# dblanm/gnn-manip

Measured on AMD Instinct MI355X. Metric: rollout steps/sec (N particles, 10 MP steps, hidden=128), higher is better.
Workload: dtype f32; 1 GPU; north_star target: N=100k dense synthetic scene, conn_r=0.015, max_neighbours=20, hidden=128, 10 MP steps; n_particles=100000, hidden=128, edges_last_step=1966056, k_steps=6, candidates_per_gpu=1, parallelism=candidate-parallel x1

## Files before the change

gnn_manip_amd/csrc/blocks_dev.h:

```cpp
#pragma once
#include "common.h"
#include "hedge.h"

namespace gm {

constexpr int kBlockEdges = 32;
__host__ __device__ inline int edge_blocks_padded(int n_edges) { return ((n_edges + kBlockEdges - 1) / kBlockEdges + 3) & ~3; }

#if defined(__HIPCC__)
__device__ inline void edge_blocks_plan(const int* __restrict__ in_ptr, int n_nodes, const int* n_per_dev, int n_per_host,
                                        EdgeBlockHeader* tab, int* gblk, int max_graphs) {
    int n_per = n_per_dev ? *n_per_dev : n_per_host;
    if (n_per <= 0) n_per = n_nodes > 0 ? n_nodes : 1;
    int G = (n_nodes + n_per - 1) / n_per;
    if (G > max_graphs) G = max_graphs;
    int pb = 0;
    for (int g = 0; g < G; ++g) {
        const int lo = g * n_per, hi = min(n_nodes, (g + 1) * n_per);
        gblk[g] = pb;
        pb += edge_blocks_padded(in_ptr[hi] - in_ptr[lo]);
    }
    gblk[G] = pb;
    tab->n_blocks = pb;
    tab->n_groups = pb / 4;
    tab->n_graphs = G;
    tab->n_per_graph = n_per;
    tab->n_stitch = 0;
}

__device__ inline void edge_blocks_fill(const int* __restrict__ in_ptr, const int* __restrict__ dst, int n_nodes, EdgeBlockHeader* tab,
                                        const int* __restrict__ gblk, int2* blk, int2* seg, int* __restrict__ head, int* __restrict__ stitch,
                                        int* __restrict__ stitch_list, int t, int nt) {
    constexpr int BE = kBlockEdges;
    const int nblk = tab->n_blocks, G = tab->n_graphs, n_per = tab->n_per_graph;
    for (int b = t; b < nblk; b += nt) {
        int lo = 0, hi = G;
        while (hi - lo > 1) {
            const int mid = (lo + hi) >> 1;
            if (gblk[mid] <= b) lo = mid; else hi = mid;
        }
        const int g = lo, j = b - gblk[g];
        const int e0 = in_ptr[g * n_per], e1 = in_ptr[min(n_nodes, (g + 1) * n_per)];
        const int start = min(e0 + j * BE, e1);
        const int cnt = min(BE, e1 - start);
        const int fl = ((j & 3) == 0 ? 1 : 0) | ((j & 3) == 3 ? 2 : 0);
        blk[b] = make_int2(start, cnt | (fl << 8));
        {
// ... 8 lines not shown
                else is_last = (j & 3) == 3 || cnt < BE || start + cnt >= e1 || dst[start + cnt] != d;
                if (is_last) last |= 1u << n;
            }
            seg[b] = make_int2((int)cont, (int)last);
        }
        if ((j & 3) == 0) {
            int h = -1;
            if (cnt > 0 && start > e0 && dst[start - 1] == dst[start]) h = dst[start];
            head[b >> 2] = h;
            if (h >= 0) {
                const int ps = start - 4 * BE;
                const bool prev_is_head = j >= 4 && dst[ps] == h && ps > e0 && dst[ps - 1] == h;
                if (!prev_is_head) {
                    stitch[h] = b >> 2;
                    stitch_list[atomicAdd(&tab->n_stitch, 1)] = h;
                }
            }
        }
    }
}
#endif

}
```

gnn_manip_amd/csrc/common.h:

```cpp
#pragma once
#include <hip/hip_runtime.h>
#include <stdint.h>
#include <stdio.h>
#include <string.h>
#include <mutex>
#include "../../include/gnn_manip_hip.h"

namespace gm {

void set_error(const char* fmt, ...);

#define GM_HIP_CHECK(expr)                                                                  \
    do {                                                                                    \
        hipError_t _e = (expr);                                                             \
        if (_e != hipSuccess) {                                                             \
            gm::set_error("%s failed: %s (%s:%d)", #expr, hipGetErrorString(_e), __FILE__,  \
                          __LINE__);                                                        \
            return GM_ERR_HIP;                                                              \
        }                                                                                   \
    } while (0)

#define GM_REQUIRE(cond, code, ...)          \
    do {                                     \
        if (!(cond)) {                       \
// ... 90 lines not shown
    size_t bytes;
};
int max_cells_for(int64_t n);
GraphWs carve_graph(void* ws, int64_t n, int max_nb);

struct CsrHeader {
    int n_edges;
    int error_flags;
    int flow;
    int pad;
};
struct CsrWs {
    CsrHeader* hdr;
    int* in_ptr;
    int* cursor;
    int* dst;
    int* src;
    int* eid;
    int* scan_in;
    int* sort_tmp;
    int64_t cap;
    int* blocks;
    size_t bytes;
};
CsrWs carve_csr(void* ws, int64_t n, int64_t cap);

enum ProfKind : int { PROF_EDGE = 0, PROF_NODE = 1, PROF_GRAPH = 2, PROF_ENC = 3, PROF_REST = 4, PROF_KINDS = 5 };
constexpr int PROF_MAX = 4096;
struct ProfState {
    int mask = 0;
// ... 114 lines not shown
```

gnn_manip_amd/csrc/graph.hip:

```cpp
#include <stdarg.h>
#include "common.h"
#include "hedge.h"
#include "blocks_dev.h"

namespace gm {

static thread_local char g_err[512] = "";
void set_error(const char* fmt, ...) {
    va_list ap;
    va_start(ap, fmt);
    vsnprintf(g_err, sizeof(g_err), fmt, ap);
    va_end(ap);
}
const char* last_error() { return g_err; }

ProfState::~ProfState() {
    for (int k = 0; k < PROF_KINDS; ++k) {
        if (!start[k]) continue;
        for (int i = 0; i < PROF_MAX; ++i) { (void)hipEventDestroy(start[k][i]); (void)hipEventDestroy(stop[k][i]); }
        delete[] start[k];
        delete[] stop[k];
    }
}

// ... 153 lines not shown
int graph_clear_jobs(StepClear& c, const GraphWs& g, int64_t n) {
    c.gh = g.hdr;
    int rc = c.add(g.cell_start, (long long)g.max_cells + 1, 0);
    if (rc == GM_OK) rc = c.add(g.cell_cursor, g.max_cells, 0);
    if (rc == GM_OK) rc = c.add(g.cnt + n, 1, 0);
    if (rc == GM_OK) rc = c.add(g.scan_cells, (long long)scan_state_ints((int64_t)g.max_cells + 1), 0);
    if (rc == GM_OK) rc = c.add(g.scan_cnt, (long long)scan_state_ints(n + 1), 0);
    return rc;
}
int csr_clear_jobs(StepClear& c, const CsrWs& w, int64_t n, int flow) {
    c.ch = w.hdr;
    c.flow = flow;
    int rc = c.add(w.in_ptr, n + 1, 0);
    if (rc == GM_OK) rc = c.add(w.scan_in, (long long)scan_state_ints(n + 1), 0);
    if (rc == GM_OK) rc = c.add(carve_edge_blocks(w.blocks, n, w.cap).stitch, n, -1);
    return rc;
}

int max_cells_for(int64_t n) {
    int64_t c = 2 * n;
    if (c < 32768) c = 32768;
    if (c > (1 << 22)) c = (1 << 22);
    return (int)c;
}

GraphWs carve_graph(void* ws, int64_t n, int max_nb) {
    GraphWs g;
    Carver c(ws);
    g.max_cells = max_cells_for(n);
    g.hdr = c.take<GraphHeader>(1);
// ... 3 lines not shown
    g.sorted = c.take<float4>(n);
    g.cnt = c.take<int>(n + 1);
    g.out_ptr = c.take<int>(n + 1);
    g.nbr = c.take<int>((size_t)n * max_nb);
    g.scan_cells = c.take<int>(scan_state_ints((int64_t)g.max_cells + 1));
    g.scan_cnt = c.take<int>(scan_state_ints(n + 1));
    g.bytes = c.used();
    return g;
}

CsrWs carve_csr(void* ws, int64_t n, int64_t cap) {
    CsrWs w;
    Carver c(ws);
    w.hdr = c.take<CsrHeader>(1);
    w.in_ptr = c.take<int>(n + 1);
    w.cursor = c.take<int>(n + 1);
    w.dst = c.take<int>(cap);
    w.src = c.take<int>(cap);
    w.eid = c.take<int>(cap);
    w.scan_in = c.take<int>(scan_state_ints(n + 1));
    w.sort_tmp = c.take<int>(2 * (size_t)cap);
    w.cap = cap;
    w.blocks = c.take<int>(edge_blocks_ints(n, cap));
    w.bytes = c.used();
    return w;
}

__device__ __forceinline__ unsigned f2ord(float f) {
    unsigned u = __float_as_uint(f);
    return (u & 0x80000000u) ? ~u : (u | 0x80000000u);
}
// ... 379 lines not shown
}

constexpr int SEG_LPS = 8;
constexpr int SEG_PER_WG = 256 / SEG_LPS;
constexpr int SEG_CAP = 96;
constexpr int SEG_STRIDE = SEG_CAP + 1;
struct BlockTabArgs {
    const int* dst;
    EdgeBlockHeader* hdr;
    const int* gblk;
    int2* blk;
    int2* seg;
    int* head;
    int* stitch;
    int* stitch_list;
    int n_tab;
};
__global__ void __launch_bounds__(256) segment_sort_kernel(const int* __restrict__ in_ptr, int64_t n,
                                                            int* __restrict__ src, int* __restrict__ eid,
                                                            CsrHeader* hdr, const float* __restrict__ pos,
                                                            int64_t pos_stride, float conn_r, float* __restrict__ edge_attr, int flow,
                                                            int* __restrict__ tmp_eid, int* __restrict__ tmp_src, BlockTabArgs bt) {
    __shared__ int se[SEG_PER_WG * SEG_STRIDE];
    __shared__ int ss[SEG_PER_WG * SEG_STRIDE];
    __shared__ int s_long[SEG_PER_WG];
    if ((int)blockIdx.x < bt.n_tab) {
        edge_blocks_fill(in_ptr, bt.dst, (int)n, bt.hdr, bt.gblk, bt.blk, bt.seg, bt.head, bt.stitch, bt.stitch_list,
                         (int)blockIdx.x * 256 + (int)threadIdx.x, bt.n_tab * 256);
        return;
    }
    const int wg = (int)blockIdx.x - bt.n_tab;
    const int tid = threadIdx.x, sub = tid & (SEG_LPS - 1), sl = tid / SEG_LPS;
    const int64_t i = (int64_t)wg * SEG_PER_WG + sl;
    if (i == 0 && sub == 0) hdr->n_edges = in_ptr[n];
    const bool active = i < n;
    const int b = active ? in_ptr[i] : 0, e = active ? in_ptr[i + 1] : 0;
    const int len = e - b;
    int* le = se + sl * SEG_STRIDE;
    int* ls = ss + sl * SEG_STRIDE;
    const bool small = len <= SEG_CAP;
    if (small)
        for (int a = sub; a < len; a += SEG_LPS) {
// ... 207 lines not shown
namespace {
int csr_tail(const GraphWs& g, int64_t n, int K, const CsrWs& c, const float* pos, int64_t pos_stride, float conn_r, float* edge_attr,
             int flow, bool with_cnt_scan, hipStream_t s) {
    const int64_t cap = n * K;
    const unsigned nb = (unsigned)cdiv(cap, 256);
    int* slot = c.sort_tmp;
    ScanJob sj[2] = {{c.in_ptr, c.in_ptr, (long long)n + 1, nullptr, c.scan_in},
                     {g.cnt, g.out_ptr, (long long)n + 1, &g.hdr->n_edges, g.scan_cnt}};
    int rc = scan_lookback(sj, with_cnt_scan ? 2 : 1, s);
    if (rc != GM_OK) return rc;
    const EdgeBlocks t = carve_edge_blocks(c.blocks, n, cap);
    hipLaunchKernelGGL(fill_graph_kernel, dim3(nb), dim3(256), 0, s, g.cnt, g.out_ptr, g.nbr, n, K, c.in_ptr,
                       slot, cap, flow, c.dst, c.src, c.eid, c.hdr, &g.hdr->n_per_graph, t.hdr, t.gblk);
    int gb = (int)cdiv(cdiv(cap, kBlockEdges) + 8, 256);
    gb = gb < 1 ? 1 : (gb > 512 ? 512 : gb);
    const BlockTabArgs bt{c.dst, t.hdr, t.gblk, t.blk, t.seg, t.head, t.stitch, t.stitch_list, gb};
    hipLaunchKernelGGL(segment_sort_kernel, dim3((unsigned)cdiv(n, SEG_PER_WG) + (unsigned)gb), dim3(256), 0, s, c.in_ptr, n, c.src, c.eid, c.hdr,
                       pos, pos_stride, conn_r, edge_attr, flow, c.sort_tmp, c.sort_tmp + c.cap, bt);
    GM_LAUNCH_CHECK();
    return GM_OK;
}
}

int csr_from_graph_with_features(const void* graph_ws, int64_t n, int K, void* csr_ws, size_t csr_ws_bytes, const float* pos,
                                 int64_t pos_stride, float conn_r, float* edge_attr, int flow, hipStream_t stream) {
    GM_REQUIRE(graph_ws && csr_ws, GM_ERR_INVALID_ARGUMENT, "gm_csr_from_graph: null pointer");
    GM_REQUIRE(flow == 0 || flow == 1, GM_ERR_INVALID_ARGUMENT, "gm_csr_from_graph: flow must be 0 or 1");
    const int64_t cap = n * K;
    GraphWs g = carve_graph(const_cast<void*>(graph_ws), n, K);
    CsrWs c = carve_csr(csr_ws, n, cap);
    GM_REQUIRE(csr_ws_bytes >= c.bytes, GM_ERR_WORKSPACE, "gm_csr_from_graph: workspace %zu < %zu", csr_ws_bytes, c.bytes);
// ... 55 lines not shown
        if (rc == GM_OK) rc = launch_step_clear(clr, s);
        if (rc != GM_OK) return rc;
    }
    if (e > 0) {
        unsigned nb = (unsigned)cdiv(e, 256);
        hipLaunchKernelGGL(indeg_ei_kernel, dim3(nb), dim3(256), 0, s, ei, n, e, flow, c.in_ptr, c.hdr);
        const ScanJob sj{c.in_ptr, c.in_ptr, (long long)n + 1, nullptr, c.scan_in};
        int rc = scan_lookback(&sj, 1, s);
        if (rc != GM_OK) return rc;
        hipLaunchKernelGGL(fill_ei_kernel, dim3(nb), dim3(256), 0, s, ei, n, e, flow, c.in_ptr, c.cursor, c.dst, c.src, c.eid, c.hdr);
    }
    if (n > 0)
        hipLaunchKernelGGL(segment_sort_kernel, dim3((unsigned)cdiv(n, SEG_PER_WG)), dim3(256), 0, s, c.in_ptr, n, c.src, c.eid, c.hdr, nullptr, 3, 1.f, nullptr, 0, c.sort_tmp, c.sort_tmp + c.cap, BlockTabArgs{});
    GM_LAUNCH_CHECK();
    if (!with_blocks) return GM_OK;
    return build_edge_blocks(c.in_ptr, c.dst, n, nullptr, (int)n, carve_edge_blocks(c.blocks, n, e), s);
}
}

extern "C" {

int gm_csr_header_status(const int32_t* header_host, int64_t* n_edges_host) {
    GM_REQUIRE(header_host, GM_ERR_INVALID_ARGUMENT, "gm_csr_header_status: null pointer");
    CsrHeader h;
    memcpy(&h, header_host, sizeof(h));
    if (n_edges_host) *n_edges_host = h.n_edges;
    GM_REQUIRE(!(h.error_flags & ERRF_BAD_EDGE_INDEX), GM_ERR_DATA, "edge_index entry out of range [0, n_nodes)");
    GM_REQUIRE(!(h.error_flags & ERRF_CAPACITY), GM_ERR_DATA, "edge capacity exceeded");
    GM_REQUIRE(!(h.error_flags & ERRF_SPLIT_RANGE), GM_ERR_DATA,
               "fp16 split range exceeded: a feature, latent or hidden activation of the last forward over this edge structure reached "
               "|x| >= 65504 in a matrix-pipe operand image (include/gnn_manip_hip.h, numeric domain); its results are not valid");
// ... 14 lines not shown
```

gnn_manip_amd/csrc/hedge.h:

```cpp
#pragma once
#include "common.h"
#include "mlp.h"

namespace gm {

struct EdgeBlockHeader {
    int n_blocks;
    int n_groups;
    int n_graphs;
    int n_per_graph;
    int n_stitch;
    int pad[3];
};
struct EdgeBlocks {
    EdgeBlockHeader* hdr;
    int* gblk;
    int2* blk;
    int2* seg;
    int* head;
    int* stitch;
    int* stitch_list;
    int64_t max_blocks;
};
size_t edge_blocks_ints(int64_t n_nodes, int64_t edge_capacity);
constexpr int kSinkRows = 1024;
size_t edge_groups_max(int64_t n_nodes, int64_t edge_capacity);
EdgeBlocks carve_edge_blocks(int* base, int64_t n_nodes, int64_t edge_capacity);
int build_edge_blocks(const int* in_ptr, const int* dst, int64_t n_nodes, const int* n_per_graph_dev, int n_per_graph_host, const EdgeBlocks& t, hipStream_t s);

constexpr int kPackH3Max = 16;
struct PackH3Job {
    const float* W1;
    int W1_col0;
    int W1_ld;
    const float* W2;
    const float* W3;
    const float* b1;
    const float* b2;
    const float* b3;
    const float* gamma;
    const float* beta;
    float* dst;
    int enc_k1;
};
size_t h3_image_floats();
int pack_h3(const PackH3Job* jobs, int n, hipStream_t s);

int launch_edge_sys(const EdgeArgs& a, const EdgeBlocks& t, int64_t edge_capacity, hipStream_t s);
inline const float* edge_sys_p_scale(const float* h3_image) { return h3_image; }

struct NodeSysArgs {
    const float* h;
    const float* agg;
    const float* Q;
    float* h_out;
    const float* image;
    int n;
    int* flags;
    float eps;
    ProfState* prof;
};
int launch_node_sys(const NodeSysArgs& a, hipStream_t s);
struct ProjSysArgs {
    const float* h;
    float* P;
    float* Q;
    const float* img_p;
    const float* img_q;
    const float* scale_p;
    const float* scale_q;
    int n;
    int* flags;
    ProfState* prof;
};
int launch_proj_sys(const ProjSysArgs& a, hipStream_t s);
int launch_agg_stitch(float* agg, const float* side, const EdgeBlocks& t, int64_t n, ProfState* prof, hipStream_t s);
constexpr int64_t kSysNodeMinNodes = 32 * 256 * 6;
int launch_edge_sys_enc(const EdgeArgs& a, hipStream_t s);
bool edge_sys_fits(int64_t n_nodes, int64_t edge_capacity);
constexpr int kEdgePadRows = 32;
int zero_edge_pad_rows(const CsrHeader* hdr, float* e, int row_floats, hipStream_t s);

}
```

gnn_manip_amd/csrc/hedge.hip:

```cpp
#include <type_traits>
#include "common.h"
#include "mlp.h"
#include "hedge.h"
#include "hmlp.h"
#include "hmma_dev.h"
#include "blocks_dev.h"

namespace gm {

namespace {

constexpr int H = 128;
constexpr int BE = 32;
constexpr int SYS_THREADS = 768;
static_assert(BE == kBlockEdges, "block tables and the systolic kernels agree on the block size");
#ifdef HEDGE_STAMPS
__device__ unsigned long long g_sys_stamps[3 * 32 * 8 + 32];
#define SYS_STAMP(tick, slot)                                                                                         \
    do {                                                                                                              \
        if (blockIdx.x == 0 && jb == 0 && lane0 == 0 && (tick) >= 16 && (tick) < 48) {                                \
            g_sys_stamps[(role * 32 + (tick) - 16) * 8 + (slot)] = __builtin_readcyclecounter();                     \
            if (role == 0 && (slot) == 0) g_sys_stamps[3 * 32 * 8 + (tick) - 16] = __builtin_amdgcn_s_memrealtime(); \
        }                                                                                                             \
    } while (0)
// ... 131 lines not shown
    switch (r) {
        case 1: scan3_t<1>(ya, yb, yc, yprev, cont); break;
        case 4: scan3_t<4>(ya, yb, yc, yprev, cont); break;
        case 7: scan3_t<7>(ya, yb, yc, yprev, cont); break;
        case 10: scan3_t<10>(ya, yb, yc, yprev, cont); break;
        default: scan3_t<13>(ya, yb, yc, yprev, cont); break;
    }
}


__device__ __forceinline__ int2 wg_range(int units, bool xcd_major) {
    const int wg = xcd_major ? xcd_major_wg() : (int)blockIdx.x;
    return make_int2((int)((long long)wg * units / gridDim.x), (int)((long long)(wg + 1) * units / gridDim.x));
}

template <class I = int>
__device__ __forceinline__ void sys_prologue(half8 (&wh)[8], half8 (&wl)[8], const half8* frag, int slice, bool one_kgroup, int zero_end, int vec_b, const float* vec, int n_vec) {
    const int tid = threadIdx.x, lane0 = tid & 63;
#pragma unroll
    for (int ks = 0; ks < 8; ++ks) {
        const int kq = one_kgroup ? 0 : ks;
        wh[ks] = frag[(((I)slice * 8 + kq) * 2 + 0) * 64 + lane0];
        wl[ks] = frag[(((I)slice * 8 + kq) * 2 + 1) * 64 + lane0];
    }
    for (int i = tid; i < zero_end / 16; i += SYS_THREADS) LDS(uintx4, i * 16) = uintx4{0u, 0u, 0u, 0u};
    for (int i = tid; i < n_vec; i += SYS_THREADS) LDS(float, vec_b + 4 * i) = vec[i];
    __builtin_amdgcn_s_waitcnt(0x0f70);
    __syncthreads();
}

__device__ __forceinline__ void set_role_prio(int role) {
    if (role == 2) __builtin_amdgcn_s_setprio(3);
    else __builtin_amdgcn_s_setprio(1);
}

__device__ __forceinline__ floatx16 vec_to_acc(char* smem, int vec_b, int f, int jb, int hi) {
    floatx16 a;
#pragma unroll
    for (int g = 0; g < 4; ++g) {
        const floatx4 v = LDS(floatx4, vec_b + (f + 32 * jb + 4 * hi + 8 * g) * 4);
#pragma unroll
// ... 488 lines not shown
    report_split_range(rng, lane0, a_flags);
}

constexpr int LN_E = 0;
constexpr int LN_X1 = LN_E + 2 * IMG_B;
constexpr int LN_X2 = LN_X1 + 2 * IMG_B;
constexpr int LN_Z = LN_X2 + 2 * IMG_B;
constexpr int LN_PS = LN_Z + 8 * TILE_B;
constexpr int LN_ST = LN_PS + 4 * TILE_B;
constexpr int LN_KM = LN_ST + 2 * 4 * 32 * 4;
constexpr int LN_ZERO_END = LN_KM + 2 * 4 * 32 * 4;
constexpr int LN_VEC = LN_ZERO_END;
constexpr size_t NODE_LDS_BYTES = LN_VEC + 4 * H * 4;
static_assert(NODE_LDS_BYTES <= 160 * 1024, "LDS budget");

__global__ void __launch_bounds__(SYS_THREADS, 1) sys_node_kernel(const float* a_h, const float* __restrict__ a_agg, const float* __restrict__ a_Q,
                                                                       float* a_h_out, const float* __restrict__ a_hw, int a_n, int* a_flags, float a_eps) {
    const int tid = threadIdx.x, lane0 = tid & 63;
    const int wave = __builtin_amdgcn_readfirstlane(tid >> 6);
    const int role = wave >> 2, jb = wave & 3;
    const int N = a_n;
    const int nblk = (N + BE - 1) / BE;
    const int wg = (int)blockIdx.x;
    const int b0 = (int)((long long)wg * nblk / gridDim.x), b1 = (int)((long long)(wg + 1) * nblk / gridDim.x);
    const int nb = b1 - b0;
    if (nb <= 0) return;
    const float inv_T = a_hw[1];
    half8 wh[8], wl[8];
    sys_prologue(wh, wl, reinterpret_cast<const half8*>(a_hw + HW_HEADER_FLOATS + HW_VEC_FLOATS), role * 4 + jb, false, LN_ZERO_END, LN_VEC,
                 a_hw + HW_HEADER_FLOATS, 4 * H);
    const int n = lane0 & 31, hi = lane0 >> 5, rr = lane0 >> 3, cq = lane0 & 7;
    const int r0 = b0 * BE;
    const int rows_wg = (b1 * BE < N ? b1 * BE : N) - r0;
    const unsigned wg_bytes = (unsigned)(rows_wg > 0 ? rows_wg : 0) * 512u;
    const unsigned v_eoff = opaque(rr * 512 + jb * 128 + cq * 16);
    int rng = 0;
    set_role_prio(role);
    if (role == 0) {
        const srd_t srd_q = make_srd(a_Q + (size_t)r0 * H, wg_bytes), srd_a = make_srd(a_agg + (size_t)r0 * H, wg_bytes);
        const unsigned v_qoff = opaque(rr * 2048 + jb * 128 + cq * 16);
        const unsigned ps_w = opaque(LN_PS + jb * TILE_B + 4 * rr * TILE_ROW_B + cq * 16);
        const unsigned ps_r = opaque(LN_PS + jb * TILE_B + n * TILE_ROW_B + hi * 16);
        const int kg = cq & 1, ksb = cq >> 2, half = (cq >> 1) & 1;
        const unsigned e_w = opaque(LN_E + ((2 * jb + ksb) * 2 * 64 + ((rr ^ (2 * (ksb + 2 * kg))) + 32 * kg)) * 16 + half * 8);
        const unsigned e_r0 = opaque(LN_E + eslot(n, hi, 0) * 16), e_r1 = opaque(LN_E + eslot(n, hi, 1) * 16);
        const unsigned x1_w = opaque(LN_X1 + 4 * jb * 1024 + lane0 * 16);
        floatx4 qv[4], eq[4];
#pragma unroll
        for (int j = 0; j < 4; ++j) { qv[j] = floatx4{0.f, 0.f, 0.f, 0.f}; eq[j] = bld4(srd_a, v_eoff, j * 4096); }
        floatx16 acc, c0v;
#pragma unroll
        for (int r = 0; r < 16; ++r) c0v[r] = 0.f;
        auto clampb = [&](int x) { return x < b0 ? b0 : (x < b1 ? x : b1 - 1); };
        auto tick = [&](auto par_c, int t) {
            constexpr int PAR = decltype(par_c)::value;
            const int x = b0 + t;
            const unsigned rel1 = (unsigned)(clampb(x + 1) - b0) * (BE * 512u), rel2 = (unsigned)(clampb(x + 2) - b0) * (BE * 512u);
#pragma unroll
            for (int j = 0; j < 4; ++j) qv[j] = bld4(srd_q, v_qoff, rel1 + j * 512);
            auto side = [&](int slot) {
                if (slot < 8 && !(slot & 1)) {
                    const int j = slot >> 1;
                    uintx2 h, l;
                    split4(eq[j][0], eq[j][1], eq[j][2], eq[j][3], h, l);
                    LDS(uintx2, e_w + (1 - PAR) * IMG_B + j * 128) = h;
                    LDS(uintx2, e_w + (1 - PAR) * IMG_B + j * 128 + 1024) = l;
                } else if (slot == 8) {
#pragma unroll
                    for (int j = 0; j < 4; ++j) eq[j] = bld4(srd_a, v_eoff, rel2 + j * 4096);
                }
            };
            mlp_layer(acc, c0v, wh, wl, smem, e_r0 + PAR * IMG_B, e_r1 + PAR * IMG_B, side);
            rng |= __any(acc[0] != acc[0]) ? 1 : 0;
            GM_SB;
            acc_to_image(acc, smem, x1_w + PAR * IMG_B);
#pragma unroll
            for (int j = 0; j < 4; ++j) LDS(floatx4, ps_w + j * TILE_ROW_B) = qv[j];
#pragma unroll
            for (int g = 0; g < 4; ++g) {
                const floatx4 v = LDS(floatx4, ps_r + 32 * g);
#pragma unroll
                for (int tt = 0; tt < 4; ++tt) c0v[4 * g + tt] = v[tt];
            }
            lds_barrier();
// ... 137 lines not shown
#pragma unroll
            for (int tt = 0; tt < 4; ++tt) z[tt] = acc[4 * g + tt] * out_scale;
            LDS(floatx4, t_w + 32 * g) = z;
        }
        const unsigned rowx = (unsigned)((x < b0 ? b0 : x) - b0) * BE;
#pragma unroll
        for (int j = 0; j < 4; ++j) {
            const floatx4 o = LDS(floatx4, t_r + j * 8 * TILE_ROW_B);
            if (isq) bst4s<ST_PROJ_Q>(make_srd(out_wg + (size_t)(rowx + 8 * j) * (out_row_b / 4), (unsigned)s_clamp0(cnt - 8 * j, 8) * out_row_b), v_out, 0, o);
            else bst4(make_srd(out_wg + (size_t)(rowx + 8 * j) * (out_row_b / 4), (unsigned)s_clamp0(cnt - 8 * j, 8) * out_row_b), v_out, 0, o);
        }
        lds_barrier();
    };
    RUN_TICKS(-1, nb, tick);
    report_split_range(rng, lane0, a_flags);
}

__global__ void __launch_bounds__(256) agg_stitch_kernel(float* __restrict__ agg, const float* __restrict__ side, const int* __restrict__ stitch,
                                                          const int* __restrict__ stitch_list, const int* __restrict__ head,
                                                          const EdgeBlockHeader* __restrict__ tab, int n) {
    const int ng = tab->n_groups, ns = tab->n_stitch;
    const int c = threadIdx.x & 7;
    for (int k = (blockIdx.x * 256 + threadIdx.x) >> 3; k < ns; k += (gridDim.x * 256) >> 3) {
        const int v = stitch_list[k];
        if (v < 0 || v >= n) continue;
        const int g0 = stitch[v];
        if (g0 < 0 || g0 >= ng || head[g0] != v) continue;
        floatx4 a[4];
#pragma unroll
        for (int q = 0; q < 4; ++q) a[q] = *reinterpret_cast<floatx4*>(agg + (size_t)v * H + 16 * c + 4 * q);
        int g = g0;
        do {
#pragma unroll
            for (int q = 0; q < 4; ++q) a[q] += *reinterpret_cast<const floatx4*>(side + (size_t)g * H + 16 * c + 4 * q);
            ++g;
        } while (g < ng && head[g] == v);
#pragma unroll
        for (int q = 0; q < 4; ++q) *reinterpret_cast<floatx4*>(agg + (size_t)v * H + 16 * c + 4 * q) = a[q];
    }
}

struct PackH3Jobs {
    int n;
    const float* W1[kPackH3Max];
    int c1[kPackH3Max];
    const float* W2[kPackH3Max];
    const float* W3[kPackH3Max];
    const float* b1[kPackH3Max];
    const float* b2[kPackH3Max];
    const float* b3[kPackH3Max];
    const float* gamma[kPackH3Max];
    const float* beta[kPackH3Max];
    float* dst[kPackH3Max];
    int enc_k1[kPackH3Max];
// ... 103 lines not shown
        const _Float16 h = (_Float16)v;
        const _Float16 lo = (_Float16)(v - (float)h);
        const size_t base = ((((size_t)(l * 4 + w) * 8 + ks) * 2) * 64 + lane) * 8 + j;
        img[base] = h;
        img[base + 64 * 8] = lo;
    }
}

__global__ void __launch_bounds__(256) edge_blocks_plan_kernel(const int* __restrict__ in_ptr, int n_nodes, const int* n_per_dev, int n_per_host,
                                                               EdgeBlockHeader* tab, int* gblk, int max_graphs) {
    if (threadIdx.x == 0) edge_blocks_plan(in_ptr, n_nodes, n_per_dev, n_per_host, tab, gblk, max_graphs);
}

__global__ void __launch_bounds__(256) edge_blocks_fill_kernel(const int* __restrict__ in_ptr, const int* __restrict__ dst, int n_nodes,
                                                               EdgeBlockHeader* tab, const int* __restrict__ gblk, int2* blk, int2* seg,
                                                               int* __restrict__ head, int* __restrict__ stitch, int* __restrict__ stitch_list) {
    edge_blocks_fill(in_ptr, dst, n_nodes, tab, gblk, blk, seg, head, stitch, stitch_list, blockIdx.x * blockDim.x + threadIdx.x,
                     gridDim.x * blockDim.x);
}

}

size_t h3_image_floats() { return (size_t)HW_HEADER_FLOATS + HW_VEC_FLOATS + (size_t)HW_IMAGE_HALF8 * 4; }

int pack_h3(const PackH3Job* jobs, int n, hipStream_t s) {
    for (int off = 0; off < n; off += kPackH3Max) {
        PackH3Jobs J{};
        J.n = n - off < kPackH3Max ? n - off : kPackH3Max;
        for (int i = 0; i < J.n; ++i) {
            const PackH3Job& j = jobs[off + i];
            J.W1[i] = j.W1; J.c1[i] = j.W1_col0; J.W2[i] = j.W2; J.W3[i] = j.W3; J.b1[i] = j.b1; J.b2[i] = j.b2; J.b3[i] = j.b3; J.gamma[i] = j.gamma; J.beta[i] = j.beta;
            J.dst[i] = j.dst;
// ... 4 lines not shown
        GM_LAUNCH_CHECK();
    }
    return GM_OK;
}

static size_t max_blocks_of(int64_t n_nodes, int64_t edge_capacity) {
    return (size_t)cdiv(edge_capacity, BE) + 4 * (size_t)n_nodes + 4;
}
size_t edge_groups_max(int64_t n_nodes, int64_t edge_capacity) { return max_blocks_of(n_nodes, edge_capacity) / 4 + 1 + kSinkRows; }

size_t edge_blocks_ints(int64_t n_nodes, int64_t edge_capacity) {
    const size_t nblk = max_blocks_of(n_nodes, edge_capacity);
    return 8 + ((size_t)n_nodes + 2) + 1 + 4 * nblk + (nblk / 4 + 2) + 2 * (size_t)n_nodes;
}

EdgeBlocks carve_edge_blocks(int* base, int64_t n_nodes, int64_t edge_capacity) {
    EdgeBlocks t;
    const size_t nblk = max_blocks_of(n_nodes, edge_capacity);
    t.hdr = reinterpret_cast<EdgeBlockHeader*>(base);
    t.gblk = base + 8;
    int* p = t.gblk + n_nodes + 2;
    p += (reinterpret_cast<uintptr_t>(p) & 4) ? 1 : 0;
    t.blk = reinterpret_cast<int2*>(p);
    t.seg = reinterpret_cast<int2*>(p + 2 * nblk);
    t.head = p + 4 * nblk;
    t.stitch = t.head + nblk / 4 + 2;
    t.stitch_list = t.stitch + n_nodes;
    t.max_blocks = (int64_t)nblk;
    return t;
}

int build_edge_blocks(const int* in_ptr, const int* dst, int64_t n_nodes, const int* n_per_graph_dev, int n_per_graph_host, const EdgeBlocks& t, hipStream_t s) {
    hipLaunchKernelGGL(edge_blocks_plan_kernel, dim3(1), dim3(64), 0, s, in_ptr, (int)n_nodes, n_per_graph_dev, n_per_graph_host,
                       t.hdr, t.gblk, (int)n_nodes + 1);
    int gb = (int)cdiv(t.max_blocks, 256);
    gb = gb < 1 ? 1 : (gb > 1024 ? 1024 : gb);
    hipLaunchKernelGGL(edge_blocks_fill_kernel, dim3(gb), dim3(256), 0, s, in_ptr, dst, (int)n_nodes, t.hdr, t.gblk, t.blk, t.seg, t.head, t.stitch,
                       t.stitch_list);
    GM_LAUNCH_CHECK();
    return GM_OK;
}

bool edge_sys_fits(int64_t n_nodes, int64_t edge_capacity) {
    const uint64_t agg_rows = (uint64_t)n_nodes + edge_groups_max(n_nodes, edge_capacity);
    return (uint64_t)n_nodes * 2 * H * 4 < (1ull << 32) && agg_rows * H * 4 < (1ull << 32);
}

constexpr uint64_t kStreamStoreBytes = 128ull << 20;

template <auto KERNEL, class... Args>
static int launch_sys(size_t lds, ProfState* prof_state, int kind, hipStream_t s, Args... args) {
    static PerDeviceOnce attr_done;
    const int rc_attr = attr_done.run([lds]() -> int {
// ... 22 lines not shown
                                                 t.blk, t.seg, t.head, t.hdr, (unsigned)(a.side - a.agg), (unsigned)agg_bytes,
                                                 (unsigned)((uint64_t)a.n_nodes_tab * 2 * H * 4), const_cast<int*>(&a.hdr->error_flags), a.eps, a.residual);
    };
    if (a.discard_e_out) return stream ? go(kernel_c<sys_edge_kernel<false, true>>{}) : go(kernel_c<sys_edge_kernel<false, false>>{});
    return stream ? go(kernel_c<sys_edge_kernel<true, true>>{}) : go(kernel_c<sys_edge_kernel<true, false>>{});
}

int launch_edge_sys_enc(const EdgeArgs& a, hipStream_t s) {
    GM_REQUIRE(a.hdr && a.wstream_h3 && a.e_in && a.e_out && !a.eid && !a.eid_out && a.k1 == 4, GM_ERR_INVALID_ARGUMENT,
               "launch_edge_sys_enc: unsupported argument combination");
    return launch_sys<sys_enc_kernel>(ENC_LDS_BYTES, a.prof, PROF_ENC, s, a.hdr, a.e_in, a.e_out, a.wstream_h3, const_cast<int*>(&a.hdr->error_flags), a.eps,
                                      a.zero_pad_rows ? 1 : 0);
}

int launch_node_sys(const NodeSysArgs& a, hipStream_t s) {
    GM_REQUIRE(a.h && a.agg && a.Q && a.h_out && a.image && a.n > 0, GM_ERR_INVALID_ARGUMENT, "launch_node_sys: bad argument");
    return launch_sys<sys_node_kernel>(NODE_LDS_BYTES, a.prof, PROF_NODE, s, a.h, a.agg, a.Q, a.h_out, a.image, a.n, a.flags, a.eps);
}

int launch_proj_sys(const ProjSysArgs& a, hipStream_t s) {
    GM_REQUIRE(a.h && a.P && a.Q && a.img_p && a.img_q && a.n > 0, GM_ERR_INVALID_ARGUMENT, "launch_proj_sys: bad argument");
    return launch_sys<sys_proj_kernel>(PROJ_LDS_BYTES, a.prof, PROF_NODE, s, a.h, a.P, a.Q, a.img_p, a.img_q, a.scale_p, a.scale_q, a.n, a.flags);
}

int launch_agg_stitch(float* agg, const float* side, const EdgeBlocks& t, int64_t n, ProfState* prof_state, hipStream_t s) {
    if (n <= 0) return GM_OK;
    {
        ProfScope prof(prof_state, PROF_NODE, s);
        int64_t gb = cdiv(n * 8, 256 * 4);
        gb = gb < 1 ? 1 : (gb > 2048 ? 2048 : gb);
        hipLaunchKernelGGL(agg_stitch_kernel, dim3((unsigned)gb), dim3(256), 0, s, agg, side, t.stitch, t.stitch_list, t.head, t.hdr, (int)n);
    }
    GM_LAUNCH_CHECK();
    return GM_OK;
}

__global__ void __launch_bounds__(256) edge_pad_rows_kernel(const CsrHeader* hdr, float* e, int row_floats) {
    const size_t base = (size_t)hdr->n_edges * row_floats;
    for (int i = blockIdx.x * blockDim.x + threadIdx.x; i < kEdgePadRows * row_floats; i += gridDim.x * blockDim.x) e[base + i] = 0.f;
}
int zero_edge_pad_rows(const CsrHeader* hdr, float* e, int row_floats, hipStream_t s) {
    hipLaunchKernelGGL(edge_pad_rows_kernel, dim3(4), dim3(256), 0, s, hdr, e, row_floats);
    GM_LAUNCH_CHECK();
    return GM_OK;
}

#ifdef HEDGE_STAMPS
extern "C" int gm_debug_sys_stamps(unsigned long long* out) {
    return hipMemcpyFromSymbol(out, HIP_SYMBOL(g_sys_stamps), sizeof(unsigned long long) * (3 * 32 * 8 + 32)) == hipSuccess ? 0 : -1;
// ... 5 lines not shown
```

gnn_manip_amd/csrc/model.hip:

```cpp
#include <algorithm>
#include <vector>
#include "common.h"
#include "mlp.h"
#include "model.h"
#include "train.h"
#include "hedge.h"
#include "hmlp.h"

using namespace gm;

std::vector<MlpSpec> gm::model_mlps(const gm_model_desc& d) {
    const int H = d.hidden_size, NL = d.num_layers;
    std::vector<MlpSpec> mlp;
    auto add = [&](int in, int out, bool normed) {
        const int base = mlp.empty() ? 0 : mlp.back().end;
        mlp.push_back({base, base + 2 * (NL + 1) + (normed ? 2 : 0), in, out, normed});
    };
    add(d.edge_dim, H, true);
    add(d.node_dim, H, true);
    for (int k = 0; k < d.m_steps; ++k) {
        add(3 * H, H, true);
        add(2 * H, H, true);
    }
    add(H, d.out_dim, false);
// ... 479 lines not shown
        rc = launch_node_hm(H, 0, na, s);
    }
    if (rc == GM_OK && route.sys_node) rc = project(0);
    if (rc != GM_OK) return rc;
    if (!agg_cleared) {
        ProfScope prof(m->prof, PROF_REST, s);
        GM_HIP_CHECK(hipMemsetAsync(f.agg, 0, (size_t)n * H * sizeof(float), s));
    }
    for (int k = 0; k < M; ++k) {
        EdgeArgs ea = proc_edge_args(m, k, c, n, nullptr, f.P, f.e, f.e, f.agg, f.side, 1);
        ea.discard_e_out = k + 1 == M;
        ea.P_prescaled = route.sys_edge;
        rc = launch_edge(H, NL, false, route.sys_edge, ea, cap, s);
        if (rc != GM_OK) return rc;
        if (route.sys_node) {
            rc = launch_agg_stitch(f.agg, f.side, carve_edge_blocks(c.blocks, n, cap), n, m->prof, s);
            NodeSysArgs ns{};
            ns.h = f.h; ns.agg = f.agg; ns.Q = f.Q; ns.h_out = f.h; ns.image = m->packed_h3 + m->h3_node[k];
            ns.n = (int)n; ns.flags = flags; ns.eps = m->d.ln_eps; ns.prof = m->prof;
            if (rc == GM_OK) rc = launch_node_sys(ns, s);
            if (rc == GM_OK && k + 1 < M) rc = project(k + 1);
            if (rc == GM_OK && k + 1 == M) rc = launch_node_hm(H, 2, tail_args(m, M, n, f.h, f.P, out, flags), s);
        } else {
            HmNodeArgs a = proc_node_args(m, k, c, n, cap, f.h, f.agg, f.side, f.h, 1);
            set_tail(m, a, k + 1, f.P, out, route.sys_edge);
            rc = launch_node_hm(H, 1, a, s);
        }
        if (rc != GM_OK) return rc;
    }
    return GM_OK;
}
}

extern "C" {

// ... 252 lines not shown
```

Baseline: 126.5 rollout steps/s.

## Fold aggregation stitch into system node kernel via per-node fold table

Removes the separate agg_stitch kernel launch and instead records a per-node fold table during edge-block building. The node kernel adds the single-group side partial sums inline when loading agg rows, and handles multi-group hub nodes during the weight-loading prologue. This saves one kernel launch and a pass over agg per message-passing step. In exchange it adds extra loads in the node kernel's load pipeline, and it aliases the fold buffer onto the cursor workspace.

```diff
diff --git a/gnn_manip_amd/csrc/blocks_dev.h b/gnn_manip_amd/csrc/blocks_dev.h
--- a/gnn_manip_amd/csrc/blocks_dev.h
+++ b/gnn_manip_amd/csrc/blocks_dev.h
@@ -28,9 +28,11 @@
     tab->n_stitch = 0;
 }
 
+__host__ __device__ inline int fold_slot(int v) { return (v & ~31) + 4 * (v & 7) + ((v >> 3) & 3); }
+__host__ __device__ inline int fold_node(int p) { return (p & ~31) + 8 * (p & 3) + ((p & 31) >> 2); }
 __device__ inline void edge_blocks_fill(const int* __restrict__ in_ptr, const int* __restrict__ dst, int n_nodes, EdgeBlockHeader* tab,
                                         const int* __restrict__ gblk, int2* blk, int2* seg, int* __restrict__ head, int* __restrict__ stitch,
-                                        int* __restrict__ stitch_list, int t, int nt) {
+                                        int* __restrict__ stitch_list, int* __restrict__ fold, int t, int nt) {
     constexpr int BE = kBlockEdges;
     const int nblk = tab->n_blocks, G = tab->n_graphs, n_per = tab->n_per_graph;
     for (int b = t; b < nblk; b += nt) {
@@ -69,6 +71,8 @@
                 if (!prev_is_head) {
                     stitch[h] = b >> 2;
                     stitch_list[atomicAdd(&tab->n_stitch, 1)] = h;
+                    const int ns = start + 4 * BE;
+                    fold[fold_slot(h)] = (ns < e1 && dst[ns] == h) ? -((b >> 2) + 1) : (b >> 2) + 1;
                 }
             }
         }
diff --git a/gnn_manip_amd/csrc/common.h b/gnn_manip_amd/csrc/common.h
--- a/gnn_manip_amd/csrc/common.h
+++ b/gnn_manip_amd/csrc/common.h
@@ -128,6 +128,7 @@
     CsrHeader* hdr;
     int* in_ptr;
     int* cursor;
+    int* fold;
     int* dst;
     int* src;
     int* eid;
diff --git a/gnn_manip_amd/csrc/graph.hip b/gnn_manip_amd/csrc/graph.hip
--- a/gnn_manip_amd/csrc/graph.hip
+++ b/gnn_manip_amd/csrc/graph.hip
@@ -1,4 +1,5 @@
 #include <stdarg.h>
+#include <algorithm>
 #include "common.h"
 #include "hedge.h"
 #include "blocks_dev.h"
@@ -191,6 +192,7 @@
     int rc = c.add(w.in_ptr, n + 1, 0);
     if (rc == GM_OK) rc = c.add(w.scan_in, (long long)scan_state_ints(n + 1), 0);
     if (rc == GM_OK) rc = c.add(carve_edge_blocks(w.blocks, n, w.cap).stitch, n, -1);
+    if (rc == GM_OK) rc = c.add(w.fold, (long long)fold_ints(n), 0);
     return rc;
 }
 
@@ -224,7 +226,8 @@
     Carver c(ws);
     w.hdr = c.take<CsrHeader>(1);
     w.in_ptr = c.take<int>(n + 1);
-    w.cursor = c.take<int>(n + 1);
+    w.cursor = c.take<int>(std::max((size_t)n + 1, fold_ints(n)));
+    w.fold = w.cursor;
     w.dst = c.take<int>(cap);
     w.src = c.take<int>(cap);
     w.eid = c.take<int>(cap);
@@ -634,6 +637,7 @@
     int* head;
     int* stitch;
     int* stitch_list;
+    int* fold;
     int n_tab;
 };
 __global__ void __launch_bounds__(256) segment_sort_kernel(const int* __restrict__ in_ptr, int64_t n,
@@ -645,7 +649,7 @@
     __shared__ int ss[SEG_PER_WG * SEG_STRIDE];
     __shared__ int s_long[SEG_PER_WG];
     if ((int)blockIdx.x < bt.n_tab) {
-        edge_blocks_fill(in_ptr, bt.dst, (int)n, bt.hdr, bt.gblk, bt.blk, bt.seg, bt.head, bt.stitch, bt.stitch_list,
+        edge_blocks_fill(in_ptr, bt.dst, (int)n, bt.hdr, bt.gblk, bt.blk, bt.seg, bt.head, bt.stitch, bt.stitch_list, bt.fold,
                          (int)blockIdx.x * 256 + (int)threadIdx.x, bt.n_tab * 256);
         return;
     }
@@ -883,7 +887,7 @@
                        slot, cap, flow, c.dst, c.src, c.eid, c.hdr, &g.hdr->n_per_graph, t.hdr, t.gblk);
     int gb = (int)cdiv(cdiv(cap, kBlockEdges) + 8, 256);
     gb = gb < 1 ? 1 : (gb > 512 ? 512 : gb);
-    const BlockTabArgs bt{c.dst, t.hdr, t.gblk, t.blk, t.seg, t.head, t.stitch, t.stitch_list, gb};
+    const BlockTabArgs bt{c.dst, t.hdr, t.gblk, t.blk, t.seg, t.head, t.stitch, t.stitch_list, c.fold, gb};
     hipLaunchKernelGGL(segment_sort_kernel, dim3((unsigned)cdiv(n, SEG_PER_WG) + (unsigned)gb), dim3(256), 0, s, c.in_ptr, n, c.src, c.eid, c.hdr,
                        pos, pos_stride, conn_r, edge_attr, flow, c.sort_tmp, c.sort_tmp + c.cap, bt);
     GM_LAUNCH_CHECK();
@@ -969,7 +973,8 @@
         hipLaunchKernelGGL(segment_sort_kernel, dim3((unsigned)cdiv(n, SEG_PER_WG)), dim3(256), 0, s, c.in_ptr, n, c.src, c.eid, c.hdr, nullptr, 3, 1.f, nullptr, 0, c.sort_tmp, c.sort_tmp + c.cap, BlockTabArgs{});
     GM_LAUNCH_CHECK();
     if (!with_blocks) return GM_OK;
-    return build_edge_blocks(c.in_ptr, c.dst, n, nullptr, (int)n, carve_edge_blocks(c.blocks, n, e), s);
+    if (n > 0) GM_HIP_CHECK(hipMemsetAsync(c.fold, 0, fold_ints(n) * sizeof(int), s));
+    return build_edge_blocks(c.in_ptr, c.dst, n, nullptr, (int)n, carve_edge_blocks(c.blocks, n, e, c.fold), s);
 }
 }
 
diff --git a/gnn_manip_amd/csrc/hedge.h b/gnn_manip_amd/csrc/hedge.h
--- a/gnn_manip_amd/csrc/hedge.h
+++ b/gnn_manip_amd/csrc/hedge.h
@@ -20,12 +20,14 @@
     int* head;
     int* stitch;
     int* stitch_list;
+    int* fold;
     int64_t max_blocks;
 };
 size_t edge_blocks_ints(int64_t n_nodes, int64_t edge_capacity);
 constexpr int kSinkRows = 1024;
 size_t edge_groups_max(int64_t n_nodes, int64_t edge_capacity);
-EdgeBlocks carve_edge_blocks(int* base, int64_t n_nodes, int64_t edge_capacity);
+EdgeBlocks carve_edge_blocks(int* base, int64_t n_nodes, int64_t edge_capacity, int* fold = nullptr);
+inline size_t fold_ints(int64_t n_nodes) { return ((size_t)n_nodes + 31) / 32 * 32; }
 int build_edge_blocks(const int* in_ptr, const int* dst, int64_t n_nodes, const int* n_per_graph_dev, int n_per_graph_host, const EdgeBlocks& t, hipStream_t s);
 
 constexpr int kPackH3Max = 16;
@@ -51,7 +53,9 @@
 
 struct NodeSysArgs {
     const float* h;
-    const float* agg;
+    float* agg;
+    const float* side;
+    EdgeBlocks tab;
     const float* Q;
     float* h_out;
     const float* image;
@@ -74,7 +78,6 @@
     ProfState* prof;
 };
 int launch_proj_sys(const ProjSysArgs& a, hipStream_t s);
-int launch_agg_stitch(float* agg, const float* side, const EdgeBlocks& t, int64_t n, ProfState* prof, hipStream_t s);
 constexpr int64_t kSysNodeMinNodes = 32 * 256 * 6;
 int launch_edge_sys_enc(const EdgeArgs& a, hipStream_t s);
 bool edge_sys_fits(int64_t n_nodes, int64_t edge_capacity);
diff --git a/gnn_manip_amd/csrc/hedge.hip b/gnn_manip_amd/csrc/hedge.hip
--- a/gnn_manip_amd/csrc/hedge.hip
+++ b/gnn_manip_amd/csrc/hedge.hip
@@ -169,8 +169,10 @@
     return make_int2((int)((long long)wg * units / gridDim.x), (int)((long long)(wg + 1) * units / gridDim.x));
 }
 
-template <class I = int>
-__device__ __forceinline__ void sys_prologue(half8 (&wh)[8], half8 (&wl)[8], const half8* frag, int slice, bool one_kgroup, int zero_end, int vec_b, const float* vec, int n_vec) {
+struct NoPrologueWork { __device__ __forceinline__ void operator()() const {} };
+template <class I = int, class F = NoPrologueWork>
+__device__ __forceinline__ void sys_prologue(half8 (&wh)[8], half8 (&wl)[8], const half8* frag, int slice, bool one_kgroup, int zero_end, int vec_b, const float* vec, int n_vec,
+                                             F&& while_loading = F{}) {
     const int tid = threadIdx.x, lane0 = tid & 63;
 #pragma unroll
     for (int ks = 0; ks < 8; ++ks) {
@@ -180,6 +182,7 @@
     }
     for (int i = tid; i < zero_end / 16; i += SYS_THREADS) LDS(uintx4, i * 16) = uintx4{0u, 0u, 0u, 0u};
     for (int i = tid; i < n_vec; i += SYS_THREADS) LDS(float, vec_b + 4 * i) = vec[i];
+    while_loading();
     __builtin_amdgcn_s_waitcnt(0x0f70);
     __syncthreads();
 }
@@ -698,8 +701,10 @@
 constexpr size_t NODE_LDS_BYTES = LN_VEC + 4 * H * 4;
 static_assert(NODE_LDS_BYTES <= 160 * 1024, "LDS budget");
 
-__global__ void __launch_bounds__(SYS_THREADS, 1) sys_node_kernel(const float* a_h, const float* __restrict__ a_agg, const float* __restrict__ a_Q,
-                                                                       float* a_h_out, const float* __restrict__ a_hw, int a_n, int* a_flags, float a_eps) {
+__global__ void __launch_bounds__(SYS_THREADS, 1) sys_node_kernel(const float* a_h, float* a_agg, const float* __restrict__ a_Q,
+                                                                       float* a_h_out, const float* __restrict__ a_hw, int a_n, int* a_flags, float a_eps,
+                                                                       const float* a_side, const int* __restrict__ a_fold, const int* __restrict__ a_head,
+                                                                       const EdgeBlockHeader* __restrict__ a_tab) {
     const int tid = threadIdx.x, lane0 = tid & 63;
     const int wave = __builtin_amdgcn_readfirstlane(tid >> 6);
     const int role = wave >> 2, jb = wave & 3;
@@ -710,18 +715,53 @@
     const int nb = b1 - b0;
     if (nb <= 0) return;
     const float inv_T = a_hw[1];
-    half8 wh[8], wl[8];
-    sys_prologue(wh, wl, reinterpret_cast<const half8*>(a_hw + HW_HEADER_FLOATS + HW_VEC_FLOATS), role * 4 + jb, false, LN_ZERO_END, LN_VEC,
-                 a_hw + HW_HEADER_FLOATS, 4 * H);
     const int n = lane0 & 31, hi = lane0 >> 5, rr = lane0 >> 3, cq = lane0 & 7;
     const int r0 = b0 * BE;
     const int rows_wg = (b1 * BE < N ? b1 * BE : N) - r0;
+    const srd_t srd_f = make_srd(a_fold + r0, (unsigned)nb * (BE * 4u));
+    const unsigned v_foff = opaque(rr * 16);
+    intx4 fq = intx4{0, 0, 0, 0}, fn = fq;
+    if (role == 0) {
+        fq = bldi4(srd_f, v_foff, 0);
+        fn = bldi4(srd_f, v_foff, nb > 1 ? BE * 4u : 0u);
+    }
+    const unsigned side_bytes = (unsigned)a_tab->n_groups * (H * 4u);
+    half8 wh[8], wl[8];
+    sys_prologue(wh, wl, reinterpret_cast<const half8*>(a_hw + HW_HEADER_FLOATS + HW_VEC_FLOATS), role * 4 + jb, false, LN_ZERO_END, LN_VEC,
+                 a_hw + HW_HEADER_FLOATS, 4 * H, [&]() {
+        const int ng = a_tab->n_groups;
+        bool rewrote = false;
+        for (int p0 = wave * 64; p0 < nb * BE; p0 += SYS_THREADS) {
+            const int f = p0 + lane0 < nb * BE ? a_fold[r0 + p0 + lane0] : 0;
+            for (unsigned long long hubs = __ballot(f < 0); hubs; hubs &= hubs - 1) {
+                const int l = __builtin_ctzll(hubs);
+                const int g0 = -__builtin_amdgcn_readlane(f, l) - 1, v = r0 + fold_node(p0 + l);
+                if (g0 >= ng || lane0 >= 32) continue;
+                float* const row = a_agg + (size_t)v * H + 4 * lane0;
+                floatx4 a = *reinterpret_cast<const floatx4*>(row);
+                int g = g0;
+                do {
+                    a += *reinterpret_cast<const floatx4*>(a_side + (size_t)g * H + 4 * lane0);
+                    ++g;
+                } while (g < ng && a_head[g] == v);
+                *reinterpret_cast<floatx4*>(row) = a;
+                rewrote = true;
+            }
+        }
+        if (__any(rewrote)) {
+            __builtin_amdgcn_s_waitcnt(0x0f70);
+            __builtin_amdgcn_fence(__ATOMIC_ACQUIRE, "agent");
+        }
+    });
     const unsigned wg_bytes = (unsigned)(rows_wg > 0 ? rows_wg : 0) * 512u;
     const unsigned v_eoff = opaque(rr * 512 + jb * 128 + cq * 16);
     int rng = 0;
     set_role_prio(role);
     if (role == 0) {
         const srd_t srd_q = make_srd(a_Q + (size_t)r0 * H, wg_bytes), srd_a = make_srd(a_agg + (size_t)r0 * H, wg_bytes);
+        const srd_t srd_s = make_srd(a_side, side_bytes);
+        const unsigned v_soff = opaque(jb * 128 + cq * 16);
+        auto side_row = [&](int j) { return bld4(srd_s, fq[j] > 0 ? ((unsigned)(fq[j] - 1) << 9) + v_soff : side_bytes, 0); };
         const unsigned v_qoff = opaque(rr * 2048 + jb * 128 + cq * 16);
         const unsigned ps_w = opaque(LN_PS + jb * TILE_B + 4 * rr * TILE_ROW_B + cq * 16);
         const unsigned ps_r = opaque(LN_PS + jb * TILE_B + n * TILE_ROW_B + hi * 16);
@@ -729,9 +769,11 @@
         const unsigned e_w = opaque(LN_E + ((2 * jb + ksb) * 2 * 64 + ((rr ^ (2 * (ksb + 2 * kg))) + 32 * kg)) * 16 + half * 8);
         const unsigned e_r0 = opaque(LN_E + eslot(n, hi, 0) * 16), e_r1 = opaque(LN_E + eslot(n, hi, 1) * 16);
         const unsigned x1_w = opaque(LN_X1 + 4 * jb * 1024 + lane0 * 16);
-        floatx4 qv[4], eq[4];
+        floatx4 qv[4], eq[4], sv[4];
 #pragma unroll
         for (int j = 0; j < 4; ++j) { qv[j] = floatx4{0.f, 0.f, 0.f, 0.f}; eq[j] = bld4(srd_a, v_eoff, j * 4096); }
+#pragma unroll
+        for (int j = 0; j < 4; ++j) sv[j] = side_row(j);
         floatx16 acc, c0v;
 #pragma unroll
         for (int r = 0; r < 16; ++r) c0v[r] = 0.f;
@@ -740,18 +782,25 @@
             constexpr int PAR = decltype(par_c)::value;
             const int x = b0 + t;
             const unsigned rel1 = (unsigned)(clampb(x + 1) - b0) * (BE * 512u), rel2 = (unsigned)(clampb(x + 2) - b0) * (BE * 512u);
+            const unsigned rel3f = (unsigned)(clampb(x + 3) - b0) * (BE * 4u);
 #pragma unroll
             for (int j = 0; j < 4; ++j) qv[j] = bld4(srd_q, v_qoff, rel1 + j * 512);
             auto side = [&](int slot) {
                 if (slot < 8 && !(slot & 1)) {
                     const int j = slot >> 1;
+                    const floatx4 st = eq[j] + sv[j];
+                    const bool has = fq[j] > 0;
                     uintx2 h, l;
-                    split4(eq[j][0], eq[j][1], eq[j][2], eq[j][3], h, l);
+                    split4(has ? st[0] : eq[j][0], has ? st[1] : eq[j][1], has ? st[2] : eq[j][2], has ? st[3] : eq[j][3], h, l);
                     LDS(uintx2, e_w + (1 - PAR) * IMG_B + j * 128) = h;
                     LDS(uintx2, e_w + (1 - PAR) * IMG_B + j * 128 + 1024) = l;
                 } else if (slot == 8) {
+                    fq = fn;
 #pragma unroll
                     for (int j = 0; j < 4; ++j) eq[j] = bld4(srd_a, v_eoff, rel2 + j * 4096);
+#pragma unroll
+                    for (int j = 0; j < 4; ++j) sv[j] = side_row(j);
+                    fn = bldi4(srd_f, v_foff, rel3f);
                 }
             };
             mlp_layer(acc, c0v, wh, wl, smem, e_r0 + PAR * IMG_B, e_r1 + PAR * IMG_B, side);
@@ -919,30 +968,6 @@
     };
     RUN_TICKS(-1, nb, tick);
     report_split_range(rng, lane0, a_flags);
-}
-
-__global__ void __launch_bounds__(256) agg_stitch_kernel(float* __restrict__ agg, const float* __restrict__ side, const int* __restrict__ stitch,
-                                                          const int* __restrict__ stitch_list, const int* __restrict__ head,
-                                                          const EdgeBlockHeader* __restrict__ tab, int n) {
-    const int ng = tab->n_groups, ns = tab->n_stitch;
-    const int c = threadIdx.x & 7;
-    for (int k = (blockIdx.x * 256 + threadIdx.x) >> 3; k < ns; k += (gridDim.x * 256) >> 3) {
-        const int v = stitch_list[k];
-        if (v < 0 || v >= n) continue;
-        const int g0 = stitch[v];
-        if (g0 < 0 || g0 >= ng || head[g0] != v) continue;
-        floatx4 a[4];
-#pragma unroll
-        for (int q = 0; q < 4; ++q) a[q] = *reinterpret_cast<floatx4*>(agg + (size_t)v * H + 16 * c + 4 * q);
-        int g = g0;
-        do {
-#pragma unroll
-            for (int q = 0; q < 4; ++q) a[q] += *reinterpret_cast<const floatx4*>(side + (size_t)g * H + 16 * c + 4 * q);
-            ++g;
-        } while (g < ng && head[g] == v);
-#pragma unroll
-        for (int q = 0; q < 4; ++q) *reinterpret_cast<floatx4*>(agg + (size_t)v * H + 16 * c + 4 * q) = a[q];
-    }
 }
 
 struct PackH3Jobs {
@@ -1076,8 +1101,9 @@
 
 __global__ void __launch_bounds__(256) edge_blocks_fill_kernel(const int* __restrict__ in_ptr, const int* __restrict__ dst, int n_nodes,
                                                                EdgeBlockHeader* tab, const int* __restrict__ gblk, int2* blk, int2* seg,
-                                                               int* __restrict__ head, int* __restrict__ stitch, int* __restrict__ stitch_list) {
-    edge_blocks_fill(in_ptr, dst, n_nodes, tab, gblk, blk, seg, head, stitch, stitch_list, blockIdx.x * blockDim.x + threadIdx.x,
+                                                               int* __restrict__ head, int* __restrict__ stitch, int* __restrict__ stitch_list,
+                                                               int* __restrict__ fold) {
+    edge_blocks_fill(in_ptr, dst, n_nodes, tab, gblk, blk, seg, head, stitch, stitch_list, fold, blockIdx.x * blockDim.x + threadIdx.x,
                      gridDim.x * blockDim.x);
 }
 
@@ -1112,7 +1138,7 @@
     return 8 + ((size_t)n_nodes + 2) + 1 + 4 * nblk + (nblk / 4 + 2) + 2 * (size_t)n_nodes;
 }
 
-EdgeBlocks carve_edge_blocks(int* base, int64_t n_nodes, int64_t edge_capacity) {
+EdgeBlocks carve_edge_blocks(int* base, int64_t n_nodes, int64_t edge_capacity, int* fold) {
     EdgeBlocks t;
     const size_t nblk = max_blocks_of(n_nodes, edge_capacity);
     t.hdr = reinterpret_cast<EdgeBlockHeader*>(base);
@@ -1124,17 +1150,19 @@
     t.head = p + 4 * nblk;
     t.stitch = t.head + nblk / 4 + 2;
     t.stitch_list = t.stitch + n_nodes;
+    t.fold = fold;
     t.max_blocks = (int64_t)nblk;
     return t;
 }
 
 int build_edge_blocks(const int* in_ptr, const int* dst, int64_t n_nodes, const int* n_per_graph_dev, int n_per_graph_host, const EdgeBlocks& t, hipStream_t s) {
+    GM_REQUIRE(t.fold, GM_ERR_INVALID_ARGUMENT, "build_edge_blocks: no fold table");
     hipLaunchKernelGGL(edge_blocks_plan_kernel, dim3(1), dim3(64), 0, s, in_ptr, (int)n_nodes, n_per_graph_dev, n_per_graph_host,
                        t.hdr, t.gblk, (int)n_nodes + 1);
     int gb = (int)cdiv(t.max_blocks, 256);
     gb = gb < 1 ? 1 : (gb > 1024 ? 1024 : gb);
     hipLaunchKernelGGL(edge_blocks_fill_kernel, dim3(gb), dim3(256), 0, s, in_ptr, dst, (int)n_nodes, t.hdr, t.gblk, t.blk, t.seg, t.head, t.stitch,
-                       t.stitch_list);
+                       t.stitch_list, t.fold);
     GM_LAUNCH_CHECK();
     return GM_OK;
 }
@@ -1187,25 +1215,14 @@
 }
 
 int launch_node_sys(const NodeSysArgs& a, hipStream_t s) {
-    GM_REQUIRE(a.h && a.agg && a.Q && a.h_out && a.image && a.n > 0, GM_ERR_INVALID_ARGUMENT, "launch_node_sys: bad argument");
-    return launch_sys<sys_node_kernel>(NODE_LDS_BYTES, a.prof, PROF_NODE, s, a.h, a.agg, a.Q, a.h_out, a.image, a.n, a.flags, a.eps);
+    GM_REQUIRE(a.h && a.agg && a.side && a.tab.hdr && a.tab.fold && a.Q && a.h_out && a.image && a.n > 0, GM_ERR_INVALID_ARGUMENT, "launch_node_sys: bad argument");
+    return launch_sys<sys_node_kernel>(NODE_LDS_BYTES, a.prof, PROF_NODE, s, a.h, a.agg, a.Q, a.h_out, a.image, a.n, a.flags, a.eps, a.side, a.tab.fold,
+                                       a.tab.head, a.tab.hdr);
 }
 
 int launch_proj_sys(const ProjSysArgs& a, hipStream_t s) {
     GM_REQUIRE(a.h && a.P && a.Q && a.img_p && a.img_q && a.n > 0, GM_ERR_INVALID_ARGUMENT, "launch_proj_sys: bad argument");
     return launch_sys<sys_proj_kernel>(PROJ_LDS_BYTES, a.prof, PROF_NODE, s, a.h, a.P, a.Q, a.img_p, a.img_q, a.scale_p, a.scale_q, a.n, a.flags);
-}
-
-int launch_agg_stitch(float* agg, const float* side, const EdgeBlocks& t, int64_t n, ProfState* prof_state, hipStream_t s) {
-    if (n <= 0) return GM_OK;
-    {
-        ProfScope prof(prof_state, PROF_NODE, s);
-        int64_t gb = cdiv(n * 8, 256 * 4);
-        gb = gb < 1 ? 1 : (gb > 2048 ? 2048 : gb);
-        hipLaunchKernelGGL(agg_stitch_kernel, dim3((unsigned)gb), dim3(256), 0, s, agg, side, t.stitch, t.stitch_list, t.head, t.hdr, (int)n);
-    }
-    GM_LAUNCH_CHECK();
-    return GM_OK;
 }
 
 __global__ void __launch_bounds__(256) edge_pad_rows_kernel(const CsrHeader* hdr, float* e, int row_floats) {
diff --git a/gnn_manip_amd/csrc/model.hip b/gnn_manip_amd/csrc/model.hip
--- a/gnn_manip_amd/csrc/model.hip
+++ b/gnn_manip_amd/csrc/model.hip
@@ -517,11 +517,11 @@
         rc = launch_edge(H, NL, false, route.sys_edge, ea, cap, s);
         if (rc != GM_OK) return rc;
         if (route.sys_node) {
-            rc = launch_agg_stitch(f.agg, f.side, carve_edge_blocks(c.blocks, n, cap), n, m->prof, s);
             NodeSysArgs ns{};
-            ns.h = f.h; ns.agg = f.agg; ns.Q = f.Q; ns.h_out = f.h; ns.image = m->packed_h3 + m->h3_node[k];
+            ns.h = f.h; ns.agg = f.agg; ns.side = f.side; ns.tab = carve_edge_blocks(c.blocks, n, cap, c.fold); ns.Q = f.Q; ns.h_out = f.h;
+            ns.image = m->packed_h3 + m->h3_node[k];
             ns.n = (int)n; ns.flags = flags; ns.eps = m->d.ln_eps; ns.prof = m->prof;
-            if (rc == GM_OK) rc = launch_node_sys(ns, s);
+            rc = launch_node_sys(ns, s);
             if (rc == GM_OK && k + 1 < M) rc = project(k + 1);
             if (rc == GM_OK && k + 1 == M) rc = launch_node_hm(H, 2, tail_args(m, M, n, f.h, f.P, out, flags), s);
         } else {
```

Measured after the change: 127.1 rollout steps/s (median of 6 runs). No clear change (+0.5%).
